# eglrp/PSBA

Measured on AMD Instinct MI355X. Metric: M-observations/sec through Jacobian+Schur build+solve (ms/LM-iter in ms_per_step), higher is better.
Workload: dtype f64; 1 GPU; venice-shaped; n_cams=52, n_pts=64053, n_obs=345364, lm=levmar, TR hand-off disabled, parallelism=points sharded x1

## Files before the change

psba_amd/csrc/kernels_linearize.hip:

```cpp
#include <cstdlib>

#include "camera_model.h"
#include "psba_internal.h"

namespace psba {

struct LinArgs {
  const double *camconst, *cams, *pts, *impts;
  const int *iidx, *jidx, *ptr;
  const int4 *tile_desc;
  double *W, *PV, *campart;
  double *camacc;
  double *dbg_ex, *dbg_JA, *dbg_JB;
  double coeff, coeff_g;
  int nC, nTiles;
  int mode;
  const double *pub_src;
  double *pub_dst;
  double pub_stamp;
  const double *kc, *wl;
  double *R;
};

template <bool DUMP, bool GACC, int LM>
__global__ __launch_bounds__(TILE_OBS) void k_linearize(LinArgs p, RobustLoss rl, FixedMask fm) {
  __shared__ double sBE[TILE_OBS][9];
  __shared__ double sW[(TILE_OBS / 2) * 19];
  extern __shared__ double sAcc[];
  const int tid = threadIdx.x;
  if (p.pub_dst && blockIdx.x == 0) {
    if (tid < NSCAL) p.pub_dst[tid] = p.pub_src[tid];
    __threadfence_system();
    __syncthreads();
    if (tid == 0) p.pub_dst[NSCAL] = p.pub_stamp;
  }
  const int nAcc = GACC ? 0 : p.nC * CAM_ACC;
  for (int t = tid; t < nAcc; t += TILE_OBS) sAcc[t] = 0.0;
  __syncthreads();

  int tile = blockIdx.x;
  int4 dsc = tile < p.nTiles ? p.tile_desc[tile] : make_int4(0, 0, 0, 0);
  int i = 0, j = 0;
  if (dsc.z + tid < dsc.w) {
    i = p.iidx[dsc.z + tid];
    j = p.jidx[dsc.z + tid];
  }
  for (; tile < p.nTiles; tile += gridDim.x) {
    const int p0 = dsc.x, p1 = dsc.y, o0 = dsc.z, o1 = dsc.w;
    const int a = o0 + tid;
    const int tn = tile + gridDim.x;
    const int4 dn = tn < p.nTiles ? p.tile_desc[tn] : make_int4(0, 0, 0, 0);
    constexpr int NTASK = (9 * TILE_PTS + TILE_OBS - 1) / TILE_OBS;
    int pb[NTASK][2];
#pragma unroll
    for (int u = 0; u < NTASK; u++) {
// ... 75 lines not shown
      for (int b = b0; b < b1; b++) {
        const double *B = sBE[b];
        acc += B[r] * B[c1] + B[3 + r] * B[c2];
      }
      p.PV[9 * (size_t)p0 + t] = (comp < 6 ? p.coeff : p.coeff_g) * acc;
    }
    if (o1 - o0 > TILE_OBS / 2) {
      __syncthreads();
      if (tid >= TILE_OBS / 2 && a < o1) {
        double *w = sW + 19 * (tid - TILE_OBS / 2);
#pragma unroll
        for (int k = 0; k < 18; k++) w[k] = Wv[k];
      }
      __syncthreads();
      if (p.mode != 2) {
        double *dst = p.W + 18 * (size_t)(o0 + TILE_OBS / 2);
        const int n = 18 * (o1 - o0 - TILE_OBS / 2);
        for (int t = tid; t < n; t += TILE_OBS) dst[t] = sW[19 * (t / 18) + t % 18];
      }
    }
    dsc = dn;
    i = j = 0;
    if (dsc.z + tid < dsc.w) {
      i = p.iidx[dsc.z + tid];
      j = p.jidx[dsc.z + tid];
    }
    __syncthreads();
  }
  if (GACC) return;
  double *slab = p.campart + (size_t)blockIdx.x * nAcc;
  for (int t = tid; t < nAcc; t += TILE_OBS) slab[t] = sAcc[t];
}

template <bool DUMP, bool GACC, int LM, bool LEAN = false>
__global__ __launch_bounds__(TILE_OBS) void k_linearize2(LinArgs p, RobustLoss rl, FixedMask fm) {
  constexpr int ROW = LEAN ? LEAN_REC + 1 : 19, REC = LEAN ? LEAN_REC : 18;
  __shared__ double sW[TILE_OBS * ROW];
  __shared__ double sCarV[TILE_OBS / 64][9];
  __shared__ int sCarP[TILE_OBS / 64][3];
  extern __shared__ double sAcc[];
  const int tid = threadIdx.x, lane = tid & 63, wave = tid >> 6;
  if (p.pub_dst && blockIdx.x == 0) {
    if (tid < NSCAL) p.pub_dst[tid] = p.pub_src[tid];
    __threadfence_system();
    __syncthreads();
    if (tid == 0) p.pub_dst[NSCAL] = p.pub_stamp;
  }
  const int nAcc = GACC || LEAN ? 0 : p.nC * CAM_ACC;
  for (int t = tid; t < nAcc; t += TILE_OBS) sAcc[t] = 0.0;
  __syncthreads();

  int tile = blockIdx.x;
  int4 dsc = tile < p.nTiles ? p.tile_desc[tile] : make_int4(0, 0, 0, 0);
  int i = 0, j = 0;
  double cc[9], cam[6], M[3], kc[5], wl[3];
  double2 m = make_double2(0.0, 0.0);
  int fx = 0;
  if (dsc.z + tid < dsc.w) {
    i = p.iidx[dsc.z + tid];
    j = p.jidx[dsc.z + tid];
    fx = fix_load<LM>(fm, i, j);
#pragma unroll
    for (int k = 0; k < 9; k++) cc[k] = p.camconst[9 * j + k];
#pragma unroll
    for (int k = 0; k < 6; k++) cam[k] = p.cams[6 * j + k];
#pragma unroll
    for (int k = 0; k < 3; k++) M[k] = p.pts[3 * (size_t)i + k];
    lens_load_kc<LM>(p.kc, j, kc);
    lens_load_w<LM>(p.wl, dsc.z + tid, wl);
    m = reinterpret_cast<const double2 *>(p.impts)[dsc.z + tid];
  }
  for (; tile < p.nTiles; tile += gridDim.x) {
    const int o0 = dsc.z, o1 = dsc.w;
    const int a = o0 + tid;
    const bool act = a < o1;
    const int tn = tile + gridDim.x;
    const int4 dn = tn < p.nTiles ? p.tile_desc[tn] : make_int4(0, 0, 0, 0);
    double v[9];
#pragma unroll
    for (int k = 0; k < 9; k++) v[k] = 0.0;
    const int pi = act ? i : -1 - tid;
    const int jc = j;
    if (act) {
      double e[2], A[12], B[6];
      lens_linearize<LM>(cc, cam, M, kc, wl, rl, m.x, m.y, e, A, B);
      fix_mask<LM>(fx, A, B);
      if (DUMP) {
        p.dbg_ex[2 * (size_t)a] = e[0];
        p.dbg_ex[2 * (size_t)a + 1] = e[1];
#pragma unroll
        for (int k = 0; k < 12; k++) p.dbg_JA[12 * (size_t)a + k] = A[k];
#pragma unroll
        for (int k = 0; k < 6; k++) p.dbg_JB[6 * (size_t)a + k] = B[k];
      }
      double *w = sW + ROW * tid;
      if (LEAN) {
#pragma unroll
        for (int k = 0; k < 12; k++) w[k] = A[k];
#pragma unroll
        for (int k = 0; k < 6; k++) w[12 + k] = B[k];
        w[18] = e[0];
        w[19] = e[1];
      } else {
#pragma unroll
        for (int r = 0; r < 6; r++)
#pragma unroll
          for (int c = 0; c < 3; c++) w[3 * r + c] = fix_w<LM>(fx, p.coeff * (A[r] * B[c] + A[6 + r] * B[3 + c]));
      }
      int q = 0;
#pragma unroll
      for (int r = 0; r < 3; r++)
#pragma unroll
        for (int c = r; c < 3; c++) v[q++] = B[r] * B[c] + B[3 + r] * B[3 + c];
#pragma unroll
      for (int r = 0; r < 3; r++) v[6 + r] = B[r] * e[0] + B[3 + r] * e[1];
      if (p.mode != 1 && !GACC && !LEAN) {
        double *acc = sAcc + CAM_ACC * (size_t)jc;
        int k = 0;
#pragma unroll
// ... 30 lines not shown
          const double vu = __shfl_up(v[k], d, 64);
          v[k] += ok ? vu : 0.0;
        }
      }
    }
    const int pn = __shfl_down(pi, 1, 64);
    const int p_first = __shfl(pi, 0, 64), p_last = __shfl(pi, 63, 64);
    if (lane == 63) {
#pragma unroll
      for (int k = 0; k < 9; k++) sCarV[wave][k] = v[k];
      sCarP[wave][0] = p_first;
      sCarP[wave][1] = p_last;
      sCarP[wave][2] = p_first == p_last;
    }
    __syncthreads();
    if (p.mode != 2) {
      double *dst = (LEAN ? p.R : p.W) + REC * (size_t)o0;
      const int n = REC * (o1 - o0);
      for (int t = tid; t < n; t += TILE_OBS) dst[t] = sW[ROW * (t / REC) + t % REC];
    }
    if (act && p.mode != 3) {
      const bool cont = lane == 63 && wave + 1 < TILE_OBS / 64 && sCarP[wave + 1][0] == pi;
      const bool tail = lane == 63 ? !cont : pn != pi;
      if (tail) {
        if (pi == p_first) {
          for (int w2 = wave - 1; w2 >= 0 && sCarP[w2][1] == pi; w2--) {
#pragma unroll
            for (int k = 0; k < 9; k++) v[k] += sCarV[w2][k];
            if (!sCarP[w2][2]) break;
          }
        }
        double *pv = p.PV + 9 * (size_t)pi;
#pragma unroll
        for (int k = 0; k < 9; k++) pv[k] = (k < 6 ? p.coeff : p.coeff_g) * v[k];
      }
    }
    dsc = dn;
    __syncthreads();
  }
  if (GACC || LEAN) return;
  double *slab = p.campart + (size_t)blockIdx.x * nAcc;
  for (int t = tid; t < nAcc; t += TILE_OBS) slab[t] = sAcc[t];
}

template <bool DUMP, bool GACC, int LM>
__global__ __launch_bounds__(TILE_OBS) void k_linearize_long(LinArgs p, const int *long_pts, double *cam_slab, RobustLoss rl, FixedMask fm) {
  __shared__ double sRed[TILE_OBS / 64][9];
  const int tid = threadIdx.x, i = long_pts[blockIdx.x];
  const int o0 = p.ptr[i], o1 = p.ptr[i + 1];
  double M[3], acc[9];
#pragma unroll
  for (int k = 0; k < 3; k++) M[k] = p.pts[3 * (size_t)i + k];
#pragma unroll
  for (int k = 0; k < 9; k++) acc[k] = 0.0;
  for (int a = o0 + tid; a < o1; a += TILE_OBS) {
    const int j = p.jidx[a];
    double cc[9], cam[6], e[2], A[12], B[6], kc[5], wl[3];
#pragma unroll
    for (int k = 0; k < 9; k++) cc[k] = p.camconst[9 * (size_t)j + k];
#pragma unroll
    for (int k = 0; k < 6; k++) cam[k] = p.cams[6 * (size_t)j + k];
    lens_load_kc<LM>(p.kc, j, kc);
    lens_load_w<LM>(p.wl, a, wl);
    const double2 m = reinterpret_cast<const double2 *>(p.impts)[a];
    lens_linearize<LM>(cc, cam, M, kc, wl, rl, m.x, m.y, e, A, B);
    const int fx = fix_load<LM>(fm, i, j);
    fix_mask<LM>(fx, A, B);
    if (DUMP) {
      p.dbg_ex[2 * (size_t)a] = e[0];
      p.dbg_ex[2 * (size_t)a + 1] = e[1];
#pragma unroll
      for (int k = 0; k < 12; k++) p.dbg_JA[12 * (size_t)a + k] = A[k];
#pragma unroll
      for (int k = 0; k < 6; k++) p.dbg_JB[6 * (size_t)a + k] = B[k];
    }
// ... 64 lines not shown
#pragma unroll
    for (int r = 0; r < 6; r++)
#pragma unroll
      for (int c = r; c < 6; c++) acc[k++] += A[r] * A[c] + A[6 + r] * A[6 + c];
#pragma unroll
    for (int r = 0; r < 6; r++) acc[21 + r] += A[r] * e[0] + A[6 + r] * e[1];
  }
#pragma unroll
  for (int k = 0; k < CAM_ACC; k++) {
#pragma unroll
    for (int d = 32; d >= 1; d >>= 1) acc[k] += __shfl_down(acc[k], d, 64);
  }
  if (lane) return;
  double *dst = p.camacc + CAM_ACC * (size_t)j;
#pragma unroll
  for (int k = 0; k < CAM_ACC; k++) atomicAdd(&dst[k], acc[k]);
}

__global__ __launch_bounds__(256) void k_cam_finalize(const double *camacc, int nC, double coeff, double coeff_g,
                                                      double *U, double *ga) {
  const int t = blockIdx.x * blockDim.x + threadIdx.x;
  if (t >= 42 * nC) return;
  const int j = t / 42, e = t % 42;
  const double *src = camacc + (size_t)j * CAM_ACC;
  if (e < 36) {
    const int r = e / 6, c = e % 6;
    const int lo = r < c ? r : c, hi = r < c ? c : r;
    U[36 * (size_t)j + e] = coeff * src[lo * 6 - lo * (lo - 1) / 2 + (hi - lo)];
  } else {
    ga[6 * (size_t)j + e - 36] = coeff_g * src[21 + e - 36];
  }
}

__global__ __launch_bounds__(1024) void k_cam_reduce(const double *campart, int nPart, int nC,
                                                     double coeff, double coeff_g, double *U,
                                                     double *ga) {
  __shared__ double sPart[32][33];
  const int j = blockIdx.x, e = threadIdx.x & 31, s = threadIdx.x >> 5;
  double acc = 0.0;
  if (e < CAM_ACC) {
    const double *src = campart + (size_t)j * CAM_ACC + e;
    const size_t stride = (size_t)nC * CAM_ACC;
    int q = s;
    for (; q + 96 < nPart; q += 128) {
      const double x0 = src[(size_t)q * stride], x1 = src[(size_t)(q + 32) * stride];
      const double x2 = src[(size_t)(q + 64) * stride], x3 = src[(size_t)(q + 96) * stride];
      acc += x0;
      acc += x1;
      acc += x2;
      acc += x3;
    }
    for (; q < nPart; q += 32) acc += src[(size_t)q * stride];
  }
  sPart[s][e] = acc;
  __syncthreads();
  if (s == 0 && e < CAM_ACC) {
    double t = sPart[0][e];
    for (int q = 1; q < 32; q++) t += sPart[q][e];
    sPart[0][e] = t;
  }
  __syncthreads();
  if (threadIdx.x < 36) {
    const int r = threadIdx.x / 6, c = threadIdx.x % 6;
    const int lo = r < c ? r : c, hi = r < c ? c : r;
    const int k = lo * 6 - lo * (lo - 1) / 2 + (hi - lo);
    U[36 * j + threadIdx.x] = coeff * sPart[0][k];
  } else if (threadIdx.x < 42) {
    ga[6 * j + threadIdx.x - 36] = coeff_g * sPart[0][21 + threadIdx.x - 36];
  }
}

__global__ __launch_bounds__(256) void k_fixed_diag(FixedMask fm, int nC, int nP, double coeff, double cam_diag, double *U,
                                                    double *ga, double *PV) {
  const int t = blockIdx.x * blockDim.x + threadIdx.x;
  if (t < nC) {
    if (fm.cams && fm.cams[t]) {
      for (int e = 0; e < 36; e++) U[36 * (size_t)t + e] = (e % 7 == 0) ? cam_diag : 0.0;
      for (int e = 0; e < 6; e++) ga[6 * (size_t)t + e] = 0.0;
    }
  } else if (t - nC < nP) {
    const int i = t - nC;
    if (fm.pts && fm.pts[i]) {
      double *pv = PV + 9 * (size_t)i;
      pv[0] = coeff; pv[1] = 0.0; pv[2] = 0.0; pv[3] = coeff; pv[4] = 0.0; pv[5] = coeff;
      pv[6] = 0.0; pv[7] = 0.0; pv[8] = 0.0;
    }
  }
}

template <int LM>
__global__ __launch_bounds__(256) void k_residual(const double *camconst, const double *cams,
                                                  const double *pts, const double *impts,
                                                  const int *iidx, const int *jidx, int nO,
                                                  double *ex_out, double *cost, const double *kcs,
                                                  const double *wls, RobustLoss rl, double *s_out) {
  __shared__ double sRed[4];
  double sum = 0.0;
  for (int a = blockIdx.x * blockDim.x + threadIdx.x; a < nO; a += gridDim.x * blockDim.x) {
    const int i = iidx[a], j = jidx[a];
    double cc[9], cam[6], M[3], e0, e1, kc[5], wl[3];
#pragma unroll
    for (int k = 0; k < 9; k++) cc[k] = camconst[9 * j + k];
// ... 39 lines not shown
              (unsigned long long)__double_as_longlong(m));
  }
}

__global__ __launch_bounds__(256) void k_max_diag_fixed(const double *U, const double *PV, int nC, int nP, double *out,
                                                        FixedMask fm) {
  __shared__ double sRed[4];
  double m = 0.0;
  const int gtid = blockIdx.x * blockDim.x + threadIdx.x, gsize = gridDim.x * blockDim.x;
  for (int t = gtid; t < 6 * nC; t += gsize)
    if (!(fm.cams && fm.cams[t / 6])) m = fmax(m, U[36 * (t / 6) + 7 * (t % 6)]);
  for (int i = gtid; i < nP; i += gsize) {
    if (fm.pts && fm.pts[i]) continue;
    const double *v = PV + 9 * (size_t)i;
    m = fmax(m, fmax(v[0], fmax(v[3], v[5])));
  }
#pragma unroll
  for (int off = 32; off > 0; off >>= 1) m = fmax(m, __shfl_down(m, off, 64));
  if ((threadIdx.x & 63) == 0) sRed[threadIdx.x >> 6] = m;
  __syncthreads();
  if (threadIdx.x == 0) {
    m = fmax(fmax(sRed[0], sRed[1]), fmax(sRed[2], sRed[3]));
    atomicMax(reinterpret_cast<unsigned long long *>(out), (unsigned long long)__double_as_longlong(m));
  }
}

template <int LM>
static int set_lin_attrs(psba_ctx *h) {
  const auto attr = hipFuncAttributeMaxDynamicSharedMemorySize;
  PSBA_HIP(h, hipFuncSetAttribute((const void *)k_linearize<true, false, LM>, attr, 100 * 1024));
  PSBA_HIP(h, hipFuncSetAttribute((const void *)k_linearize<false, false, LM>, attr, 100 * 1024));
  PSBA_HIP(h, hipFuncSetAttribute((const void *)k_linearize2<true, false, LM>, attr, 100 * 1024));
  PSBA_HIP(h, hipFuncSetAttribute((const void *)k_linearize2<false, false, LM>, attr, 100 * 1024));
  return PSBA_OK;
}

template <int LM>
static void enqueue_linearize(psba_ctx *h, const LinArgs &a, const RobustLoss &rl, const FixedMask &fm, bool dump, bool v1, size_t lds, double *Uo, double *gao) {
  const Dims &d = h->d;
  if (h->cam_global) {
    const int grid = d.nTiles < 2048 ? d.nTiles : 2048;
    if (v1 && dump)
      hipLaunchKernelGGL((k_linearize<true, true, LM>), dim3(grid), dim3(TILE_OBS), 0, h->stream, a, rl, fm);
    else if (v1)
      hipLaunchKernelGGL((k_linearize<false, true, LM>), dim3(grid), dim3(TILE_OBS), 0, h->stream, a, rl, fm);
    else if (dump)
      hipLaunchKernelGGL((k_linearize2<true, true, LM>), dim3(grid), dim3(TILE_OBS), 0, h->stream, a, rl, fm);
    else
      hipLaunchKernelGGL((k_linearize2<false, true, LM>), dim3(grid), dim3(TILE_OBS), 0, h->stream, a, rl, fm);
    if (h->nLong) {
      if (dump)
        hipLaunchKernelGGL((k_linearize_long<true, true, LM>), dim3(h->nLong), dim3(TILE_OBS), 0, h->stream, a, h->long_pts, (double *)nullptr, rl, fm);
      else
        hipLaunchKernelGGL((k_linearize_long<false, true, LM>), dim3(h->nLong), dim3(TILE_OBS), 0, h->stream, a, h->long_pts, (double *)nullptr, rl, fm);
    }
    hipLaunchKernelGGL(k_cam_sums<LM>, dim3((h->nCamUnits + 3) / 4), dim3(256), 0, h->stream, a, h->cam_obs,
                       h->cam_units, h->nCamUnits, rl, fm);
    hipLaunchKernelGGL(k_cam_finalize, dim3((42 * d.nC + 255) / 256), dim3(256), 0, h->stream, h->camacc, d.nC,
                       h->coeff, h->coeff_g, Uo, gao);
  } else {
    if (v1 && dump)
      hipLaunchKernelGGL((k_linearize<true, false, LM>), dim3(h->nPart), dim3(TILE_OBS), lds, h->stream, a, rl, fm);
    else if (v1)
      hipLaunchKernelGGL((k_linearize<false, false, LM>), dim3(h->nPart), dim3(TILE_OBS), lds, h->stream, a, rl, fm);
    else if (dump)
      hipLaunchKernelGGL((k_linearize2<true, false, LM>), dim3(h->nPart), dim3(TILE_OBS), lds, h->stream, a, rl, fm);
    else
      hipLaunchKernelGGL((k_linearize2<false, false, LM>), dim3(h->nPart), dim3(TILE_OBS), lds, h->stream, a, rl, fm);
    int nslab = h->nPart;
    if (h->nLong) {
      double *slab = h->campart + (size_t)h->nPart * d.nC * CAM_ACC;
      if (dump)
        hipLaunchKernelGGL((k_linearize_long<true, false, LM>), dim3(h->nLong), dim3(TILE_OBS), 0, h->stream, a, h->long_pts, slab, rl, fm);
      else
        hipLaunchKernelGGL((k_linearize_long<false, false, LM>), dim3(h->nLong), dim3(TILE_OBS), 0, h->stream, a, h->long_pts, slab, rl, fm);
      nslab++;
    }
    hipLaunchKernelGGL(k_cam_reduce, dim3(d.nC), dim3(1024), 0, h->stream, h->campart, nslab, d.nC, h->coeff,
                       h->coeff_g, Uo, gao);
  }
}

int launch_linearize(psba_ctx *h, bool dump, bool ahead, bool publish, bool lean) {
  if (h->cnp != 6) return dump ? mirror_refused(h) : launch_linearize_free(h, ahead, publish);
  (ahead ? h->lean_alt : h->lean_cur) = lean;
  const Dims &d = h->d;
  LinArgs a;
  a.camconst = h->camconst;
  const int set = ahead ? 1 - h->cur : h->cur;
  a.cams = h->cams[set];
  a.pts = h->pts[set];
  a.impts = h->impts;
  a.iidx = h->iidx;
  a.jidx = h->jidx;
  a.ptr = h->ptr;
  a.tile_desc = h->tile_desc;
  a.W = ahead ? h->W_alt : h->W;
  a.PV = ahead ? h->PV_alt : h->PV;
  a.campart = h->campart;
  a.camacc = h->camacc;
  a.dbg_ex = h->dbg_ex;
  a.dbg_JA = h->dbg_JA;
  a.dbg_JB = h->dbg_JB;
  a.coeff = h->coeff;
  h->coeff_w = h->coeff;
  a.coeff_g = h->coeff_g;
  a.nC = d.nC;
  a.nTiles = d.nTiles;
  a.pub_src = h->scal;
  a.pub_dst = publish ? h->h_scal_dev : nullptr;
  a.pub_stamp = h->pub_seq;
  a.kc = h->lens_kc;
  a.wl = h->lens_w;
  a.R = ahead ? h->R_alt : h->R;
  const RobustLoss rl = make_robust_loss(h->loss_kind, h->loss_c);
  const FixedMask fm = {h->fix_cams, h->fix_pts};
  if (lean) {
    a.mode = 0;
    ProfScope ps(h, PSBA_K_LINEARIZE);
    hipLaunchKernelGGL((k_linearize2<false, false, LENS_PLAIN, true>), dim3(h->nPart), dim3(TILE_OBS), 0, h->stream, a, rl, fm);
    PSBA_HIP(h, hipGetLastError());
    return PSBA_OK;
  }
  {
    const char *m = getenv("PSBA_LIN_MODE");
    a.mode = m ? atoi(m) : 0;
  }
  const bool v1 = getenv("PSBA_LIN_V1") != nullptr;
  const size_t lds = h->cam_global ? 0 : sizeof(double) * CAM_ACC * (size_t)d.nC;
  if (!h->lin_attr_set && lds > 8 * 1024) {
    int rc = PSBA_OK;
    for (int lm = 0; lm < 2 * LENS_MODELS && rc == PSBA_OK; lm++)
      lens_dispatch_fixed(lm % LENS_MODELS, lm >= LENS_MODELS, [&](auto m) { rc = set_lin_attrs<decltype(m)::value>(h); });
    if (rc != PSBA_OK) return rc;
    h->lin_attr_set = true;
  }
  double *Uo = ahead ? h->U_alt : h->U, *gao = ahead ? h->ga_alt : h->ga;
  {
    ProfScope ps(h, PSBA_K_LINEARIZE);
    if (h->cam_global)
      PSBA_HIP(h, hipMemsetAsync(h->camacc, 0, sizeof(double) * CAM_ACC * (size_t)d.nC, h->stream));
    else if (h->nLong)
      PSBA_HIP(h, hipMemsetAsync(h->campart + (size_t)h->nPart * d.nC * CAM_ACC, 0, sizeof(double) * CAM_ACC * (size_t)d.nC,
                                 h->stream));
    lens_dispatch_fixed(h->lens, h->has_fixed, [&](auto m) { enqueue_linearize<decltype(m)::value>(h, a, rl, fm, dump, v1, lds, Uo, gao); });
    if (h->has_fixed)
      hipLaunchKernelGGL(k_fixed_diag, dim3((d.nC + d.nP + 255) / 256), dim3(256), 0, h->stream, fm, d.nC, d.nP, h->coeff,
                         h->rank == 0 ? h->coeff : 0.0, Uo, gao, a.PV);
  }
  PSBA_HIP(h, hipGetLastError());
  return PSBA_OK;
}

int launch_residual(psba_ctx *h, int which, double *ex_out_dev, double *s_out_dev) {
  if (h->cnp != 6) return ex_out_dev || s_out_dev ? mirror_refused(h) : launch_residual_free(h, which);
  const Dims &d = h->d;
  const int set = which == PSBA_PARAMS_NEW ? 1 - h->cur : h->cur;
  PSBA_HIP(h, hipMemsetAsync(h->scal + SC_COST, 0, sizeof(double), h->stream));
  int grid = (d.nO + 255) / 256;
  if (grid > 256) grid = 256;
  {
    ProfScope ps(h, PSBA_K_RESIDUAL);
    const RobustLoss rl = make_robust_loss(h->loss_kind, h->loss_c);
    lens_dispatch(h->lens | (s_out_dev ? LENS_ROBUST : 0), [&](auto m) {
      hipLaunchKernelGGL(k_residual<decltype(m)::value>, dim3(grid), dim3(256), 0, h->stream, h->camconst, h->cams[set],
                         h->pts[set], h->impts, h->iidx, h->jidx, d.nO, ex_out_dev, h->scal + SC_COST, h->lens_kc,
                         h->lens_w, rl, s_out_dev);
    });
  }
  PSBA_HIP(h, hipGetLastError());
  return PSBA_OK;
}

int launch_max_diag(psba_ctx *h) {
  if (h->cnp != 6) return launch_max_diag_free(h);
  PSBA_HIP(h, hipMemsetAsync(h->scal + SC_MAXDIAG, 0, sizeof(double), h->stream));
  int grid = (h->d.nP + 255) / 256;
  if (grid > 512) grid = 512;
  if (h->has_fixed)
    hipLaunchKernelGGL(k_max_diag_fixed, dim3(grid), dim3(256), 0, h->stream, h->U, h->PV, h->d.nC, h->d.nP,
                       h->scal + SC_MAXDIAG, FixedMask{h->fix_cams, h->fix_pts});
  else
    hipLaunchKernelGGL(k_max_diag, dim3(grid), dim3(256), 0, h->stream, h->U, h->PV, h->d.nC, h->d.nP,
                       h->scal + SC_MAXDIAG);
  PSBA_HIP(h, hipGetLastError());
  return PSBA_OK;
}

}
```

psba_amd/csrc/psba_api.cpp:

```cpp
#include <algorithm>
#include <cmath>
#include <cstdarg>
#include <cstdio>
#include <cstdlib>
#include <cstring>
#include <string>
#include <new>
#include <vector>

#include "api_common.h"
#include "camera_model.h"

using namespace psba;

static thread_local std::string g_create_err;

namespace psba {

int fail(psba_ctx *h, int code, const char *fmt, ...) {
  char buf[1024];
  va_list ap;
  va_start(ap, fmt);
  vsnprintf(buf, sizeof buf, fmt, ap);
  va_end(ap);
// ... 61 lines not shown

extern "C" {

const char *psba_version(void) { return "psba_hip 0.1 (gfx950, fp64)"; }

const char *psba_last_error(psba_handle h) { return h ? h->err.c_str() : g_create_err.c_str(); }

static hipError_t create_main_stream(hipStream_t *s) {
  int least = 0, greatest = 0;
  if (getenv("PSBA_STREAM_PRIO_DEFAULT") || hipDeviceGetStreamPriorityRange(&least, &greatest) != hipSuccess)
    return hipStreamCreateWithFlags(s, hipStreamNonBlocking);
  return hipStreamCreateWithPriority(s, hipStreamNonBlocking, greatest);
}

int psba_create(int device, psba_handle *out) {
  if (!out) return PSBA_E_INVALID;
  *out = nullptr;
  int ndev = 0;
  hipError_t e = hipGetDeviceCount(&ndev);
  if (e != hipSuccess || ndev == 0)
    return fail(nullptr, PSBA_E_HIP, "no HIP device available (%s); this library has no CPU path",
                e == hipSuccess ? "device count 0" : hipGetErrorString(e));
  if (device < 0 || device >= ndev)
    return fail(nullptr, PSBA_E_INVALID, "device %d out of range (%d devices)", device, ndev);
  psba_ctx *h = new psba_ctx();
  h->device = device;
  if ((e = hipSetDevice(device)) != hipSuccess ||
      (e = create_main_stream(&h->stream)) != hipSuccess ||
      (e = hipEventCreateWithFlags(&h->scal_event, hipEventDisableTiming)) != hipSuccess) {
    int rc = fail(nullptr, PSBA_E_HIP, "psba_create: %s", hipGetErrorString(e));
    psba_destroy(h);
    return rc;
  }
  if (h->scal.alloc(h, NSCAL) != PSBA_OK || h->h_scal.alloc(h, NSCAL + 8) != PSBA_OK) {
    int rc = fail(nullptr, PSBA_E_HIP, "psba_create: %s", h->err.c_str());
    psba_destroy(h);
    return rc;
  }
  if (hipHostGetDevicePointer((void **)&h->h_scal_dev, h->h_scal, 0) != hipSuccess) h->h_scal_dev = nullptr;
  h->status = reinterpret_cast<int *>(h->scal + 8);
  h->h_status = reinterpret_cast<int *>(h->h_scal + 8);
  (void)hipMemsetAsync(h->scal, 0, sizeof(double) * NSCAL, h->stream);
  (void)hipStreamSynchronize(h->stream);
  h->h_scal[NSCAL] = 0.0;
  *out = h;
  return PSBA_OK;
}

int psba_destroy(psba_handle h) {
  CHECK_H(h);
  (void)hipSetDevice(h->device);
  if (h->stream) (void)hipStreamSynchronize(h->stream);
  if (h->stream2) (void)hipStreamSynchronize(h->stream2);
  if (h->comm) ncclCommDestroy(h->comm);
  if (h->k3_event) (void)hipEventDestroy(h->k3_event);
  for (hipEvent_t e : h->chol_events) (void)hipEventDestroy(e);
  if (h->chol_side) {
    (void)hipStreamSynchronize(h->chol_side);
    (void)hipStreamDestroy(h->chol_side);
  }
  if (h->stream2) (void)hipStreamDestroy(h->stream2);
  if (h->scal_event) (void)hipEventDestroy(h->scal_event);
  for (auto &s : h->spans) {
    (void)hipEventDestroy(s.a);
    (void)hipEventDestroy(s.b);
  }
  if (h->stream) (void)hipStreamDestroy(h->stream);
  delete h;
  return PSBA_OK;
}

int psba_schur_path(psba_handle h, int *path) {
  CHECK_H(h);
  NEED(h, h->uploaded, "no problem uploaded");
  if (path) *path = h->cnp != 6 ? 5 : h->solver == PSBA_SOLVER_PCG ? 4 : getenv("PSBA_SCHUR_ATOMIC") ? 2 : h->ring_nWg > 0 ? 3 : h->nGroups > 0 ? 0 : 1;
// ... 386 lines not shown
    }
    cams = cam11.data();
  }
  auto H2D = [&](void *dst, const void *src, size_t bytes) {
    return hipMemcpyAsync(dst, src, bytes, hipMemcpyHostToDevice, h->stream);
  };
  PSBA_HIP(h, H2D(h->cams[0], cams, sizeof(double) * d.nA));
  PSBA_HIP(h, H2D(h->pts[0], u.pts3D, sizeof(double) * d.nB));
  PSBA_HIP(h, H2D(h->params0, cams, sizeof(double) * d.nA));
  PSBA_HIP(h, H2D(h->params0 + d.nA, u.pts3D, sizeof(double) * d.nB));
  PSBA_HIP(h, H2D(h->impts, u.impts, sizeof(double) * 2 * (size_t)d.nO));
  PSBA_HIP(h, H2D(h->iidx, u.iidx, sizeof(int) * (size_t)d.nO));
  PSBA_HIP(h, H2D(h->jidx, u.jidx, sizeof(int) * (size_t)d.nO));
  PSBA_HIP(h, hipStreamSynchronize(h->stream));
  return PSBA_OK;
}

int psba_upload_problem(psba_handle h, int nCams, int n3Dpts, int n2Dprojs, const double *Kparas,
                        const double *impts, const double *initrot, const double *camsEx,
                        const double *pts3D, const int *iidx, const int *jidx) {
  CHECK_H(h);
  Upload u{nCams, n3Dpts, n2Dprojs, Kparas, impts, initrot, camsEx, pts3D, iidx, jidx};
  TRY(build_point_csr(h, u));
  cut_tiles(u);
  PSBA_HIP(h, hipSetDevice(h->device));
  drop_problem(h);
  set_dims(h, u);
  TRY(alloc_work_buffers(h));
  if (h->cam_global || h->cnp != 6) TRY(upload_camera_index(h, u));
  TRY(plan_schur(h, u));
  h->lean_ok = h->cnp == 6 && h->solver != PSBA_SOLVER_PCG && h->nGroups > 0 && h->ring_nWg == 0 && !h->schur_runs &&
               !h->schur_pairs && !h->cam_global && h->nLong == 0;
  if (const char *e = getenv("PSBA_LEAN_LIN")) h->lean_ok = h->lean_ok && atoi(e) != 0;
  TRY(copy_inputs(h, u));
  PSBA_HIP(h, hipDeviceSynchronize());
  h->uploaded = true;
  return PSBA_OK;
}

static void abandon_try(psba_ctx *h) { h->backsub_pending = h->publish_deferred = h->publish_in_k1 = false; }

int psba_set_params(psba_handle h, const double *camsEx, const double *pts3D) {
  CHECK_H(h);
  NEED(h, h->uploaded, "no problem uploaded");
  if (!h->kd_rep_h.empty()) TRY(groups_split(h, "psba_set_params", h->kd_rep_h, camsEx, KD_CNP, 10, 0));
  PSBA_HIP(h, hipMemcpyAsync(h->cams[h->cur], camsEx, sizeof(double) * h->d.nA,
                             hipMemcpyHostToDevice, h->stream));
  PSBA_HIP(h, hipMemcpyAsync(h->pts[h->cur], pts3D, sizeof(double) * h->d.nB,
                             hipMemcpyHostToDevice, h->stream));
  PSBA_HIP(h, hipStreamSynchronize(h->stream));
  params_changed(h);
  abandon_try(h);
  return PSBA_OK;
}

int psba_reset_params(psba_handle h) {
  CHECK_H(h);
  NEED(h, h->uploaded, "no problem uploaded");
  PSBA_HIP(h, hipMemcpyAsync(h->cams[h->cur], h->params0, sizeof(double) * h->d.nA, hipMemcpyDeviceToDevice,
                             h->stream));
  PSBA_HIP(h, hipMemcpyAsync(h->pts[h->cur], h->params0 + h->d.nA, sizeof(double) * h->d.nB,
                             hipMemcpyDeviceToDevice, h->stream));
  params_changed(h);
  abandon_try(h);
  return PSBA_OK;
}
// ... 42 lines not shown
  NEED(h, h->uploaded, "no problem uploaded");
  if (!(h->lin_is_ahead && coeff == h->coeff && coeff_g == h->coeff_g)) {
    h->coeff = coeff;
    h->coeff_g = coeff_g;
    TRY(launch_linearize(h, false));
    h->free_obs = h->cnp != 6;
    h->damp_ok = h->damp_kind == PSBA_DAMPING_MARQUARDT;
  }
  h->lin_is_ahead = false;
  h->ahead = false;
  h->linearized = true;
  h->assembled = h->solved = h->backsubbed = false;
  return PSBA_OK;
}

static int enqueue_max_diag(psba_ctx *h) {
  if (h->comm) {
    double *tmp = h->dp;
    PSBA_HIP(h, hipMemcpyAsync(tmp, h->U, sizeof(double) * 36 * h->d.nC, hipMemcpyDeviceToDevice,
                               h->stream));
    RCCL(h, ncclAllReduce(tmp, tmp, (size_t)36 * h->d.nC, ncclDouble, ncclSum, h->comm, h->stream));
    std::swap(h->U, h->dp);
    int rc = launch_max_diag(h);
    std::swap(h->U, h->dp);
    TRY(rc);
    RCCL(h, ncclAllReduce(h->scal + SC_MAXDIAG, h->scal + SC_MAXDIAG, 1, ncclDouble, ncclMax,
                          h->comm, h->stream));
  } else {
    TRY(launch_max_diag(h));
  }
  return PSBA_OK;
}

int psba_begin(psba_handle h, double coeff, double coeff_g, double *cost, double *max_diag) {
  CHECK_H(h);
  NEED(h, h->uploaded, "no problem uploaded");
  TRY(enqueue_residual(h, PSBA_PARAMS_CUR));
  h->coeff = coeff;
  h->coeff_g = coeff_g;
  TRY(launch_linearize(h, false));
  h->free_obs = h->cnp != 6;
  h->damp_ok = h->damp_kind == PSBA_DAMPING_MARQUARDT;
  h->linearized = true;
  h->assembled = h->solved = h->backsubbed = false;
  h->ahead = false;
  TRY(enqueue_max_diag(h));
  TRY(fetch_scalars(h));
  if (cost) *cost = h->h_scal[SC_COST];
  if (max_diag) *max_diag = h->h_scal[SC_MAXDIAG];
  h->lin_is_ahead = true;
  return PSBA_OK;
}

int psba_max_diag(psba_handle h, double *out) {
  CHECK_H(h);
  NEED(h, h->linearized, "psba_linearize first");
  TRY(enqueue_max_diag(h));
  TRY(fetch_scalars(h));
  if (out) *out = h->h_scal[SC_MAXDIAG];
  return PSBA_OK;
}

int psba_schur_assemble(psba_handle h, double mu) {
  CHECK_H(h);
  NEED(h, h->linearized, "psba_linearize first");
  h->mu = mu;
  h->try_shortcut = h->struct_only && h->cnp == 6 && !getenv("PSBA_FIXED_NO_SHORTCUT");
  h->cholmod_factor = false;
  if (h->try_shortcut)
// ... 140 lines not shown
  h->lean_cur = h->lean_alt = false;
  return PSBA_OK;
}

}
}

int psba_linearize_ahead(psba_handle h) { return linearize_ahead(h, false); }

int psba_linearize_lean(psba_handle h) {
  CHECK_H(h);
  NEED(h, h->linearized, "psba_linearize first");
  NEED(h, !h->backsub_pending, "a damping try is in flight (psba_backsub_wait first)");
  NEED(h, lean_prepare(h), "this handle takes the standard form only (psba_lm_ran_lean in include/psba_hip.h lists what the lean form needs)");
  TRY(launch_linearize(h, false, false, false, true));
  h->assembled = h->solved = h->backsubbed = false;
  return PSBA_OK;
}

int psba_lm_ran_lean(psba_handle h, int *lean) {
  CHECK_H(h);
  if (lean) *lean = h->lm_lean ? 1 : 0;
  return PSBA_OK;
}

int psba_backsub_wait(psba_handle h, psba_try_scalars *out) {
  CHECK_H_NOJOIN(h);
  NEED(h, h->backsub_pending, "psba_backsub_async first");
  if (h->publish_deferred) {
    TRY(publish_scalars(h, h->stream));
    h->publish_deferred = false;
  }
  if (h->publish_in_k1) {
    volatile double *stamp = h->h_scal + NSCAL;
    long long spin = 0;
    while (*stamp != h->pub_seq && ++spin < 200000000LL) {
      if ((spin & 0xfffff) == 0 && hipStreamQuery(h->stream) != hipErrorNotReady) break;
    }
    if (*stamp != h->pub_seq) {
      PSBA_HIP(h, hipStreamSynchronize(h->stream));
      if (*stamp != h->pub_seq) return fail(h, PSBA_E_HIP, "the try's scalars did not reach the host");
    }
    __sync_synchronize();
    h->publish_in_k1 = false;
  } else {
    for (int spin = 0; spin < 20000 && hipEventQuery(h->scal_event) == hipErrorNotReady; spin++) {
    }
    PSBA_HIP(h, hipEventSynchronize(h->scal_event));
  }
  h->scal_side = false;
  h->backsub_pending = false;
  for (int q = 0; q < 4; q++) {
    double v = 0.0;
    for (int s = 0; s < SC_NPART; s++) v += h->h_scal[SC_PART + 4 * s + q];
    h->h_scal[SC_DP_L2 + q] = v;
  }
  const int st0 = h->h_scal[SC_STATUS_V] > 0.0 ? h->try_id : 0;
  const int st1 = h->h_scal[SC_STATUS_SPD] > 0.0 ? h->try_id : 0;
  h->backsubbed = true;
  if (out) {
    out->status = (st1 == h->try_id ? PSBA_NOT_SPD : 0) | (st0 == h->try_id ? PSBA_SINGULAR_V : 0);
    out->dp_l2 = h->h_scal[SC_DP_L2];
    out->gain_den = h->h_scal[SC_GAIN_DEN];
    out->new_cost = h->h_scal[SC_NEW_COST];
    out->newp_l2 = h->h_scal[SC_NEWP_L2];
  }
  return PSBA_OK;
}

int psba_backsub(psba_handle h, double mu, psba_try_scalars *out) {
  TRY(psba_backsub_async(h, mu));
  return psba_backsub_wait(h, out);
}

int psba_accept(psba_handle h) {
  CHECK_H(h);
// ... 917 lines not shown
```

psba_amd/csrc/psba_internal.h:

```cpp
#pragma once
#include <hip/hip_runtime.h>
#include <rccl/rccl.h>

#include <string>
#include <vector>

#include "../../include/psba_hip.h"
#include "dev_buf.h"

namespace psba {

constexpr int TILE_OBS = 256;
constexpr int TILE_PTS = 128;
constexpr int MAX_GROUPS = 128;
constexpr int CAM_ACC = 27;
constexpr int LEAN_REC = 20;
constexpr int NSCAL = 104;
constexpr int SC_NPART = 16;

enum {
  SC_COST = 0,
  SC_DP_L2 = 1,
  SC_GAIN_DEN = 2,
  SC_NEW_COST = 3,
  SC_NEWP_L2 = 4,
  SC_MAXDIAG = 7,
  SC_PART = 16,
  SC_STATUS_V = 80,
  SC_STATUS_SPD = 81,
  SC_TR_DOTS = 84,
  SC_CHOLMOD = 88,
  SC_SUMS = 96,
};

struct Dims {
  int nC = 0, nP = 0, nO = 0;
  int nA = 0, nB = 0, nT = 0;
  int nTiles = 0;
  int nTilesAll = 0;
  int maxTrack = 0;
};

constexpr int ITEM_OBS_BITS = 24, ITEM_PT_BITS = 22, ITEM_BOFF_BITS = 8, ITEM_POS_BITS = 10;
struct SchurWg {
  int group, nblk;
  int obs0, pt0;
  long long item0, item1;
  unsigned long long slab_off;
  long long itemD;
};
constexpr int PAIR_OBS_BITS = 18, PAIR_PT_BITS = 16;
constexpr unsigned long long SCHUR_NULL_ITEM = ~0ull;
struct ReduceGroup {
  int nwg, nblk;
  long long pos0;
  unsigned long long slab;
  unsigned long long pad;
};

// ... 77 lines not shown
}

struct ProblemState {
  psba::Dims d;
  psba::DevBuf<double> camconst;
  psba::DevBuf<double> cams[2];
  psba::DevBuf<double> pts[2];
  psba::DevBuf<double> params0;
  psba::DevBuf<double> impts;
  int lens = 0;
  int loss_kind = 0;
  double loss_c = 1.0;
  psba::DevBuf<double> obs_s;
  psba::DevBuf<double> lens_kc;
  psba::DevBuf<double> lens_w;
  psba::DevBuf<unsigned char> fix_cams, fix_pts;
  int n_fix_cams = 0, n_fix_pts = 0;
  bool has_fixed = false, struct_only = false;
  bool try_shortcut = false;
  psba::DevBuf<int> iidx;
  psba::DevBuf<int> jidx;
  psba::DevBuf<int> ptr;
  psba::DevBuf<int> tile_pt;
  psba::DevBuf<int> long_pts;
  int nLong = 0;
  psba::DevBuf<int4> tile_desc;
  psba::DevBuf<double> W;
  psba::DevBuf<double> PV;
  psba::DevBuf<double> U;
  psba::DevBuf<double> ga;
  psba::DevBuf<double> W_alt, PV_alt, U_alt, ga_alt;
  psba::DevBuf<double> R, R_alt;
  bool lean_ok = false, lean_cur = false, lean_alt = false, lm_lean = false;
  bool ahead = false;
  bool lin_is_ahead = false;
  bool scal_side = false;
  psba::DevBuf<double> campart;
  int nPart = 0;
  bool cam_global = false;
  psba::DevBuf<double> camacc;
  psba::DevBuf<int> cam_obs;
  psba::DevBuf<int4> cam_units;
  int nCamUnits = 0;
  psba::DevBuf<double> red;
  int n32 = 0;
  int nGroups = 0;
  int nWg = 0;
  std::vector<int> gblk0;
  std::vector<int> gnwg;
  std::vector<int> gnblk;
  std::vector<size_t> gslab;
  psba::DevBuf<psba::ReduceGroup> gtab;
  psba::DevBuf<psba::SchurWg> wg;
  psba::DevBuf<unsigned long long> items;
  bool schur_runs = false;
  bool schur_pairs = false;
  psba::DevBuf<double> redp;
  size_t packed_doubles = 0;
  bool packed_pending = false;
  psba::DevBuf<double> diag0;
  int h_diagpos[21] = {0};
  int h_diaggrp[21] = {0};
  bool diag_done = false;
  bool cholmod_factor = false;
  psba::DevBuf<int> posblock;
  psba::DevBuf<double> slab;
// ... 92 lines not shown
  bool uploaded = false, linearized = false, assembled = false, solved = false, backsubbed = false;
  bool backsub_pending = false;
  bool free_obs = false;
  bool publish_deferred = false, publish_in_k1 = false;
  int cur = 0;
  double coeff = 1.0, coeff_g = 1.0, mu = 0.0;
  double coeff_w = 1.0;
  bool mu_applied = false;
};

struct psba_ctx : ProblemState {
  int device = 0;
  hipStream_t stream = nullptr;
  std::string err;

  ncclComm_t comm = nullptr;
  int nranks = 1, rank = 0;

  double *h_scal_dev = nullptr;
  hipEvent_t scal_event = nullptr;
  hipStream_t stream2 = nullptr;
  hipEvent_t k3_event = nullptr;
  hipStream_t chol_side = nullptr;
  std::vector<hipEvent_t> chol_events;

  int solver = 0;
  int cnp = 6;
  double pcg_tol = 1e-10;
  int pcg_maxit = 500;
  psba::PinnedBuf<double> pcg_host;
  std::vector<unsigned char> bs_pattern;

  psba::DevBuf<double> scal;
  int *status = nullptr;
  int try_id = 0;
  double pub_seq = 0.0;
  psba::PinnedBuf<double> h_scal;
  int *h_status = nullptr;

  bool lds_attr_set = false, atomic_attr_set = false, chol_attr_set = false, lin_attr_set = false, ring_attr_set = false;

  unsigned prof = 0;
  struct Span { hipEvent_t a, b; int kind; };
  std::vector<Span> spans;
  size_t spans_used = 0;
  double prof_ms[PSBA_K_COUNT] = {0};
  int prof_n[PSBA_K_COUNT] = {0};
};

namespace psba {

int fail(psba_ctx *h, int code, const char *fmt, ...);
bool lean_eligible(psba_ctx *h);
bool lean_prepare(psba_ctx *h);
int linearize_ahead(psba_ctx *h, bool lean);
int lean_restore(psba_ctx *h);
#define PSBA_HIP(h, call)                                                              \
  do {                                                                                 \
    hipError_t e__ = (call);                                                           \
    if (e__ != hipSuccess)                                                             \
      return psba::fail((h), PSBA_E_HIP, "%s failed: %s (%s:%d)", #call,               \
                        hipGetErrorString(e__), __FILE__, __LINE__);                   \
  } while (0)

struct ProfScope {
  psba_ctx *h;
  int idx = -1;
  ProfScope(psba_ctx *h, int kind);
  ~ProfScope();
};

int launch_linearize(psba_ctx *h, bool dump, bool ahead = false, bool publish = false, bool lean = false);
int launch_residual(psba_ctx *h, int which, double *ex_out_dev, double *s_out_dev = nullptr);
int launch_max_diag(psba_ctx *h);
int build_schur_plan(psba_ctx *h, int nCams, int nPts, int nObs, const int *iidx, const int *jidx,
                     const int *ptr, SchurPlanHost &out);
int build_owner_plan(int nCams, int nObs, const int *iidx, const int *jidx, const int *ptr, OwnerPlanHost &out,
                     const unsigned char *pattern = nullptr);
int sparse_pattern(int nCams, int nObs, const int *iidx, const int *jidx, const int *ptr, unsigned char *flags);
#ifdef PSBA_BUILD_EXPERIMENTS
int build_ring_plan(int nCams, int nPts, int nObs, const int *iidx, const int *jidx, const int *ptr, RingPlanHost &out,
                    bool force = false);
int launch_schur_ring(psba_ctx *h, double mu, bool dump);
struct SchurLdsArgs;
bool launch_schur_lds_mode(int mode, dim3 G, dim3 B, size_t lds, hipStream_t s, const SchurLdsArgs &a);
#endif
int launch_schur(psba_ctx *h, double mu, bool dump);
int launch_schur_expand(psba_ctx *h);
int launch_chol_solve(psba_ctx *h);
int mirror_refused(psba_ctx *h);
int build_blockprod_plan(int nCams, int nObs, const int *iidx, const int *jidx, const int *ptr, int seg_len,
                         BlockProdPlanHost &out);
int launch_linearize_free(psba_ctx *h, bool ahead, bool publish);
int launch_residual_free(psba_ctx *h, int which);
int launch_obs_weights_free(psba_ctx *h, int which, double *s_dev, double *w_dev);
int launch_prior_cost_free(psba_ctx *h, int which, double *out2_dev);
int launch_max_diag_free(psba_ctx *h);
int launch_schur_free(psba_ctx *h, double mu);
int launch_backsub_free(psba_ctx *h, double mu);
int launch_bsr_finalize(psba_ctx *h, double mu);
int launch_pcg_solve(psba_ctx *h);
int launch_bsr_gershgorin(psba_ctx *h, double *lambda, double *info3);
int launch_bsr_times(psba_ctx *h, const double *x_host, double *y_host);
int launch_chol_graph(psba_ctx *h);
int chol_dist_shape(psba_ctx *h, int *NB, int *blocked);
// ... 20 lines not shown
```

Before: 2262 M-obs/s.

## Fuse begin-step cost and max-diagonal into single linearize pass

psba_begin now runs one linearize kernel that also accumulates the robust cost and the largest diagonal entry, instead of a separate residual pass, a linearize and a max-diag kernel. Partial sums and the max go through atomics into a small buffer that a tiny kernel publishes to pinned host memory, and the host spins on a stamp. This is meant to cut kernel launches and a redundant read of the observations at the start of each solve. It recomputes the residual inside linearize, which adds some arithmetic, and it applies only to the plain lens model with no fixed parameters on a single rank.

```diff
diff --git a/psba_amd/csrc/kernels_linearize.hip b/psba_amd/csrc/kernels_linearize.hip
--- a/psba_amd/csrc/kernels_linearize.hip
+++ b/psba_amd/csrc/kernels_linearize.hip
@@ -20,7 +20,12 @@
   double pub_stamp;
   const double *kc, *wl;
   double *R;
+  double *begin_acc;
 };
+
+__device__ __forceinline__ void begin_max(double *dst, double m) {
+  atomicMax(reinterpret_cast<unsigned long long *>(dst), (unsigned long long)__double_as_longlong(m));
+}
 
 template <bool DUMP, bool GACC, int LM>
 __global__ __launch_bounds__(TILE_OBS) void k_linearize(LinArgs p, RobustLoss rl, FixedMask fm) {
@@ -162,7 +167,7 @@
   for (int t = tid; t < nAcc; t += TILE_OBS) slab[t] = sAcc[t];
 }
 
-template <bool DUMP, bool GACC, int LM, bool LEAN = false>
+template <bool DUMP, bool GACC, int LM, bool LEAN = false, bool BEGIN = false>
 __global__ __launch_bounds__(TILE_OBS) void k_linearize2(LinArgs p, RobustLoss rl, FixedMask fm) {
   constexpr int ROW = LEAN ? LEAN_REC + 1 : 19, REC = LEAN ? LEAN_REC : 18;
   __shared__ double sW[TILE_OBS * ROW];
@@ -186,6 +191,7 @@
   double cc[9], cam[6], M[3], kc[5], wl[3];
   double2 m = make_double2(0.0, 0.0);
   int fx = 0;
+  double bcost = 0.0, bmax = 0.0;
   if (dsc.z + tid < dsc.w) {
     i = p.iidx[dsc.z + tid];
     j = p.jidx[dsc.z + tid];
@@ -215,6 +221,11 @@
       double e[2], A[12], B[6];
       lens_linearize<LM>(cc, cam, M, kc, wl, rl, m.x, m.y, e, A, B);
       fix_mask<LM>(fx, A, B);
+      if (BEGIN) {
+        double r0, r1;
+        lens_residual<LM>(cc, cam, M, kc, wl, m.x, m.y, r0, r1);
+        bcost += lens_cost<LM>(rl, r0, r1);
+      }
       if (DUMP) {
         p.dbg_ex[2 * (size_t)a] = e[0];
         p.dbg_ex[2 * (size_t)a + 1] = e[1];
@@ -311,7 +322,11 @@
         }
         double *pv = p.PV + 9 * (size_t)pi;
 #pragma unroll
-        for (int k = 0; k < 9; k++) pv[k] = (k < 6 ? p.coeff : p.coeff_g) * v[k];
+        for (int k = 0; k < 9; k++) {
+          const double s = (k < 6 ? p.coeff : p.coeff_g) * v[k];
+          pv[k] = s;
+          if (BEGIN && (k == 0 || k == 3 || k == 5)) bmax = fmax(bmax, s);
+        }
       }
     }
     dsc = dn;
@@ -320,6 +335,27 @@
   if (GACC || LEAN) return;
   double *slab = p.campart + (size_t)blockIdx.x * nAcc;
   for (int t = tid; t < nAcc; t += TILE_OBS) slab[t] = sAcc[t];
+  if (BEGIN) {
+#pragma unroll
+    for (int off = 32; off > 0; off >>= 1) {
+      bcost += __shfl_down(bcost, off, 64);
+      bmax = fmax(bmax, __shfl_down(bmax, off, 64));
+    }
+    if (lane == 0) {
+      sCarV[wave][0] = bcost;
+      sCarV[wave][1] = bmax;
+    }
+    __syncthreads();
+    if (tid == 0) {
+      double c = 0.0, m = 0.0;
+      for (int w2 = 0; w2 < TILE_OBS / 64; w2++) {
+        c += sCarV[w2][0];
+        m = fmax(m, sCarV[w2][1]);
+      }
+      atomicAdd(&p.begin_acc[blockIdx.x % BEGIN_NPART], c);
+      begin_max(p.begin_acc + BEGIN_NPART, m);
+    }
+  }
 }
 
 template <bool DUMP, bool GACC, int LM>
@@ -450,9 +486,10 @@
   }
 }
 
+template <bool BEGIN = false>
 __global__ __launch_bounds__(1024) void k_cam_reduce(const double *campart, int nPart, int nC,
                                                      double coeff, double coeff_g, double *U,
-                                                     double *ga) {
+                                                     double *ga, double *begin_acc = nullptr) {
   __shared__ double sPart[32][33];
   const int j = blockIdx.x, e = threadIdx.x & 31, s = threadIdx.x >> 5;
   double acc = 0.0;
@@ -485,7 +522,25 @@
     U[36 * j + threadIdx.x] = coeff * sPart[0][k];
   } else if (threadIdx.x < 42) {
     ga[6 * j + threadIdx.x - 36] = coeff_g * sPart[0][21 + threadIdx.x - 36];
-  }
+  } else if (BEGIN && threadIdx.x == 64) {
+    double m = 0.0;
+#pragma unroll
+    for (int r = 0; r < 6; r++) m = fmax(m, coeff * sPart[0][r * 6 - r * (r - 1) / 2]);
+    begin_max(begin_acc + BEGIN_NPART, m);
+  }
+}
+
+__global__ __launch_bounds__(64) void k_publish_begin(double *acc, double *host, double stamp) {
+  if (threadIdx.x == 0) {
+    double c = 0.0;
+    for (int s = 0; s < BEGIN_NPART; s++) c += acc[s];
+    host[SC_BEGIN_COST] = c;
+    host[SC_BEGIN_MAX] = acc[BEGIN_NPART];
+  }
+  __threadfence_system();
+  __syncthreads();
+  if (threadIdx.x == 0) host[NSCAL] = stamp;
+  if (threadIdx.x <= BEGIN_NPART) acc[threadIdx.x] = 0.0;
 }
 
 __global__ __launch_bounds__(256) void k_fixed_diag(FixedMask fm, int nC, int nP, double coeff, double cam_diag, double *U,
@@ -591,12 +646,22 @@
   PSBA_HIP(h, hipFuncSetAttribute((const void *)k_linearize<false, false, LM>, attr, 100 * 1024));
   PSBA_HIP(h, hipFuncSetAttribute((const void *)k_linearize2<true, false, LM>, attr, 100 * 1024));
   PSBA_HIP(h, hipFuncSetAttribute((const void *)k_linearize2<false, false, LM>, attr, 100 * 1024));
+  if constexpr (LM == LENS_PLAIN)
+    PSBA_HIP(h, hipFuncSetAttribute((const void *)k_linearize2<false, false, LENS_PLAIN, false, true>, attr, 100 * 1024));
   return PSBA_OK;
 }
 
 template <int LM>
-static void enqueue_linearize(psba_ctx *h, const LinArgs &a, const RobustLoss &rl, const FixedMask &fm, bool dump, bool v1, size_t lds, double *Uo, double *gao) {
+static void enqueue_linearize(psba_ctx *h, const LinArgs &a, const RobustLoss &rl, const FixedMask &fm, bool dump, bool v1, size_t lds, double *Uo, double *gao, bool begin) {
   const Dims &d = h->d;
+  if constexpr (LM == LENS_PLAIN) {
+    if (begin) {
+      hipLaunchKernelGGL((k_linearize2<false, false, LENS_PLAIN, false, true>), dim3(h->nPart), dim3(TILE_OBS), lds, h->stream, a, rl, fm);
+      hipLaunchKernelGGL(k_cam_reduce<true>, dim3(d.nC), dim3(1024), 0, h->stream, h->campart, h->nPart, d.nC, h->coeff,
+                         h->coeff_g, Uo, gao, a.begin_acc);
+      return;
+    }
+  }
   if (h->cam_global) {
     const int grid = d.nTiles < 2048 ? d.nTiles : 2048;
     if (v1 && dump)
@@ -635,12 +700,12 @@
         hipLaunchKernelGGL((k_linearize_long<false, false, LM>), dim3(h->nLong), dim3(TILE_OBS), 0, h->stream, a, h->long_pts, slab, rl, fm);
       nslab++;
     }
-    hipLaunchKernelGGL(k_cam_reduce, dim3(d.nC), dim3(1024), 0, h->stream, h->campart, nslab, d.nC, h->coeff,
-                       h->coeff_g, Uo, gao);
-  }
-}
-
-int launch_linearize(psba_ctx *h, bool dump, bool ahead, bool publish, bool lean) {
+    hipLaunchKernelGGL(k_cam_reduce<false>, dim3(d.nC), dim3(1024), 0, h->stream, h->campart, nslab, d.nC, h->coeff,
+                       h->coeff_g, Uo, gao, (double *)nullptr);
+  }
+}
+
+int launch_linearize(psba_ctx *h, bool dump, bool ahead, bool publish, bool lean, bool begin) {
   if (h->cnp != 6) return dump ? mirror_refused(h) : launch_linearize_free(h, ahead, publish);
   (ahead ? h->lean_alt : h->lean_cur) = lean;
   const Dims &d = h->d;
@@ -672,6 +737,7 @@
   a.kc = h->lens_kc;
   a.wl = h->lens_w;
   a.R = ahead ? h->R_alt : h->R;
+  a.begin_acc = h->begin_acc;
   const RobustLoss rl = make_robust_loss(h->loss_kind, h->loss_c);
   const FixedMask fm = {h->fix_cams, h->fix_pts};
   if (lean) {
@@ -702,7 +768,7 @@
     else if (h->nLong)
       PSBA_HIP(h, hipMemsetAsync(h->campart + (size_t)h->nPart * d.nC * CAM_ACC, 0, sizeof(double) * CAM_ACC * (size_t)d.nC,
                                  h->stream));
-    lens_dispatch_fixed(h->lens, h->has_fixed, [&](auto m) { enqueue_linearize<decltype(m)::value>(h, a, rl, fm, dump, v1, lds, Uo, gao); });
+    lens_dispatch_fixed(h->lens, h->has_fixed, [&](auto m) { enqueue_linearize<decltype(m)::value>(h, a, rl, fm, dump, v1, lds, Uo, gao, begin); });
     if (h->has_fixed)
       hipLaunchKernelGGL(k_fixed_diag, dim3((d.nC + d.nP + 255) / 256), dim3(256), 0, h->stream, fm, d.nC, d.nP, h->coeff,
                          h->rank == 0 ? h->coeff : 0.0, Uo, gao, a.PV);
@@ -731,6 +797,12 @@
   return PSBA_OK;
 }
 
+int launch_publish_begin(psba_ctx *h) {
+  hipLaunchKernelGGL(k_publish_begin, dim3(1), dim3(64), 0, h->stream, h->begin_acc.get(), h->h_scal_dev, h->pub_seq);
+  PSBA_HIP(h, hipGetLastError());
+  return PSBA_OK;
+}
+
 int launch_max_diag(psba_ctx *h) {
   if (h->cnp != 6) return launch_max_diag_free(h);
   PSBA_HIP(h, hipMemsetAsync(h->scal + SC_MAXDIAG, 0, sizeof(double), h->stream));
diff --git a/psba_amd/csrc/psba_api.cpp b/psba_amd/csrc/psba_api.cpp
--- a/psba_amd/csrc/psba_api.cpp
+++ b/psba_amd/csrc/psba_api.cpp
@@ -117,7 +117,8 @@
     psba_destroy(h);
     return rc;
   }
-  if (h->scal.alloc(h, NSCAL) != PSBA_OK || h->h_scal.alloc(h, NSCAL + 8) != PSBA_OK) {
+  if (h->scal.alloc(h, NSCAL) != PSBA_OK || h->h_scal.alloc(h, NSCAL + 8) != PSBA_OK ||
+      h->begin_acc.alloc(h, BEGIN_NPART + 1) != PSBA_OK) {
     int rc = fail(nullptr, PSBA_E_HIP, "psba_create: %s", h->err.c_str());
     psba_destroy(h);
     return rc;
@@ -126,6 +127,7 @@
   h->status = reinterpret_cast<int *>(h->scal + 8);
   h->h_status = reinterpret_cast<int *>(h->h_scal + 8);
   (void)hipMemsetAsync(h->scal, 0, sizeof(double) * NSCAL, h->stream);
+  (void)hipMemsetAsync(h->begin_acc, 0, sizeof(double) * (BEGIN_NPART + 1), h->stream);
   (void)hipStreamSynchronize(h->stream);
   h->h_scal[NSCAL] = 0.0;
   *out = h;
@@ -578,6 +580,8 @@
   h->lean_ok = h->cnp == 6 && h->solver != PSBA_SOLVER_PCG && h->nGroups > 0 && h->ring_nWg == 0 && !h->schur_runs &&
                !h->schur_pairs && !h->cam_global && h->nLong == 0;
   if (const char *e = getenv("PSBA_LEAN_LIN")) h->lean_ok = h->lean_ok && atoi(e) != 0;
+  h->begin_ok = h->cnp == 6 && !h->cam_global && h->nLong == 0;
+  if (const char *e = getenv("PSBA_BEGIN_ONE_PASS")) h->begin_ok = h->begin_ok && atoi(e) != 0;
   TRY(copy_inputs(h, u));
   PSBA_HIP(h, hipDeviceSynchronize());
   h->uploaded = true;
@@ -686,9 +690,45 @@
   return PSBA_OK;
 }
 
+static int wait_stamp(psba_ctx *h, const char *what) {
+  volatile double *stamp = h->h_scal + NSCAL;
+  long long spin = 0;
+  while (*stamp != h->pub_seq && ++spin < 200000000LL) {
+    if ((spin & 0xfffff) == 0 && hipStreamQuery(h->stream) != hipErrorNotReady) break;
+  }
+  if (*stamp != h->pub_seq) {
+    PSBA_HIP(h, hipStreamSynchronize(h->stream));
+    if (*stamp != h->pub_seq) return fail(h, PSBA_E_HIP, "%s did not reach the host", what);
+  }
+  __sync_synchronize();
+  return PSBA_OK;
+}
+
+static bool begin_one_pass(psba_ctx *h) {
+  return h->begin_ok && h->h_scal_dev && !h->comm && h->nranks == 1 && h->lens == 0 && !h->has_fixed &&
+         !getenv("PSBA_LIN_V1") && !getenv("PSBA_LIN_MODE");
+}
+
 int psba_begin(psba_handle h, double coeff, double coeff_g, double *cost, double *max_diag) {
   CHECK_H(h);
   NEED(h, h->uploaded, "no problem uploaded");
+  if (begin_one_pass(h)) {
+    h->coeff = coeff;
+    h->coeff_g = coeff_g;
+    TRY(launch_linearize(h, false, false, false, false, true));
+    h->free_obs = false;
+    h->damp_ok = h->damp_kind == PSBA_DAMPING_MARQUARDT;
+    h->linearized = true;
+    h->assembled = h->solved = h->backsubbed = false;
+    h->ahead = false;
+    h->pub_seq += 1.0;
+    TRY(launch_publish_begin(h));
+    TRY(wait_stamp(h, "psba_begin's cost and largest diagonal entry"));
+    if (cost) *cost = h->h_scal[SC_BEGIN_COST];
+    if (max_diag) *max_diag = h->h_scal[SC_BEGIN_MAX];
+    h->lin_is_ahead = true;
+    return PSBA_OK;
+  }
   TRY(enqueue_residual(h, PSBA_PARAMS_CUR));
   h->coeff = coeff;
   h->coeff_g = coeff_g;
@@ -895,16 +935,7 @@
     h->publish_deferred = false;
   }
   if (h->publish_in_k1) {
-    volatile double *stamp = h->h_scal + NSCAL;
-    long long spin = 0;
-    while (*stamp != h->pub_seq && ++spin < 200000000LL) {
-      if ((spin & 0xfffff) == 0 && hipStreamQuery(h->stream) != hipErrorNotReady) break;
-    }
-    if (*stamp != h->pub_seq) {
-      PSBA_HIP(h, hipStreamSynchronize(h->stream));
-      if (*stamp != h->pub_seq) return fail(h, PSBA_E_HIP, "the try's scalars did not reach the host");
-    }
-    __sync_synchronize();
+    TRY(wait_stamp(h, "the try's scalars"));
     h->publish_in_k1 = false;
   } else {
     for (int spin = 0; spin < 20000 && hipEventQuery(h->scal_event) == hipErrorNotReady; spin++) {
diff --git a/psba_amd/csrc/psba_internal.h b/psba_amd/csrc/psba_internal.h
--- a/psba_amd/csrc/psba_internal.h
+++ b/psba_amd/csrc/psba_internal.h
@@ -17,6 +17,7 @@
 constexpr int LEAN_REC = 20;
 constexpr int NSCAL = 104;
 constexpr int SC_NPART = 16;
+constexpr int BEGIN_NPART = 16;
 
 enum {
   SC_COST = 0,
@@ -25,6 +26,8 @@
   SC_NEW_COST = 3,
   SC_NEWP_L2 = 4,
   SC_MAXDIAG = 7,
+  SC_BEGIN_COST = 10,
+  SC_BEGIN_MAX = 11,
   SC_PART = 16,
   SC_STATUS_V = 80,
   SC_STATUS_SPD = 81,
@@ -168,6 +171,7 @@
   psba::DevBuf<double> W_alt, PV_alt, U_alt, ga_alt;
   psba::DevBuf<double> R, R_alt;
   bool lean_ok = false, lean_cur = false, lean_alt = false, lm_lean = false;
+  bool begin_ok = false;
   bool ahead = false;
   bool lin_is_ahead = false;
   bool scal_side = false;
@@ -326,6 +330,7 @@
   std::vector<unsigned char> bs_pattern;
 
   psba::DevBuf<double> scal;
+  psba::DevBuf<double> begin_acc;
   int *status = nullptr;
   int try_id = 0;
   double pub_seq = 0.0;
@@ -364,7 +369,8 @@
   ~ProfScope();
 };
 
-int launch_linearize(psba_ctx *h, bool dump, bool ahead = false, bool publish = false, bool lean = false);
+int launch_linearize(psba_ctx *h, bool dump, bool ahead = false, bool publish = false, bool lean = false, bool begin = false);
+int launch_publish_begin(psba_ctx *h);
 int launch_residual(psba_ctx *h, int which, double *ex_out_dev, double *s_out_dev = nullptr);
 int launch_max_diag(psba_ctx *h);
 int build_schur_plan(psba_ctx *h, int nCams, int nPts, int nObs, const int *iidx, const int *jidx,
```

New measurement: 2284 M-obs/s, median of 3. No clear change (+1.0%).
